# marcinmiklitz/pywindow

Hardware: AMD Instinct MI355X
Metric: trajectory frames/sec full_analysis (pore+windows), CC3 1k-frame (higher is better)
Workload: dtype f64

## Files before the change

pywindow_amd/csrc/pw_unit.hpp:

```cpp
#pragma once
#include "../../include/pywindow_amd.h"
#include "pw_lbfgsb.hpp"
#include "pw_math.hpp"
#include "pw_team.hpp"
#include <string.h>

#if defined(PW_PROFILE) && defined(__HIPCC__)
__shared__ unsigned long long pw_prof_lds[32];
#define PW_PROF_BASE(ws) ((unsigned long long*)pw_prof_lds)
#endif
#if defined(PW_PROFILE) && defined(__HIP_DEVICE_COMPILE__)
#define PW_T0(var) long long var = wall_clock64()
#if defined(PW_ZPROF) && defined(PW_LB_FINE)
#define PW_T1(ws, slot, var) do { (void)var; } while (0)
#elif defined(PW_BARRIER_PROF)
#define PW_T1(ws, slot, var) do { (void)var; if (T::lane() == 0) { unsigned long long w_ = 0; \
        for (int k_ = 0; k_ < T::NWAVES; ++k_) w_ += atomicExch(&pw_bar_acc[k_], 0ull); \
        atomicAdd(&pw_prof_lds[slot], w_); } } while (0)
#else
#define PW_T1(ws, slot, var) do { if (T::lane() == 0) atomicAdd(&pw_prof_lds[slot], (unsigned long long)(wall_clock64() - var)); } while (0)
#endif
#else
#define PW_T0(var) do {} while (0)
#define PW_T1(ws, slot, var) do {} while (0)
#endif

namespace pw {

constexpr double GOLDEN_ANGLE = 2.399963229728653;
constexpr double FOUR_PI = 12.566370614359172;
constexpr double FOUR_THIRDS_PI = 4.1887902047863905;
constexpr double TWO_PI = 6.283185307179586;
constexpr double ONE_PI = 3.141592653589793;

constexpr int PW_KCLS = 8;
#ifndef PW_LEFTOVER_ROUND_DIV
#define PW_LEFTOVER_ROUND_DIV 16
#endif
constexpr double PW_PATH_POINTS_MAX = 1048576.0;
struct ClassInfo {
    int k;
    int off[PW_KCLS + 1];
    double vdw[PW_KCLS];
};
struct Frame {
    ldouble *x, *y, *z, *xx;
    const ldouble* vdw;
    const lint* perm;
    const PW_LDS ClassInfo* cls;
};

struct TeamWorkspace {
    double* knn;
    double* pts;
    double* vals;
    int* surv_k;
    int* labels;
    unsigned char* flag;
    unsigned long long* adj;
    double* xw;
    int* xw_ok;
    int p_cap;
    const unsigned* nb_off;
    const unsigned short* nb_idx;
    const double* nb_unit;
    const double* nb_bound;
    pw_extra_window* xwin;
    unsigned* xwin_count;
    unsigned xwin_cap;
    double leaf[256];
    double acc8[8 * 160];
    int leaf_tab[324];
    unsigned long long prof[32];
    const unsigned* rsq;
    pw_unit_debug* dbg_base;
    long unit;
};
PW_HD inline size_t team_slab_bytes(int p_cap) { return (size_t)p_cap * 192; }
PW_HD inline size_t team_adj_words(int p_cap) { return (size_t)p_cap * (size_t)(p_cap / 64); }
PW_HD inline int round_p_cap(long p) {
    if (p < PW_P_MAX) p = PW_P_MAX;
    return (int)((p + 127) & ~127l);
}
PW_HD inline int params_p_cap(double adjust_windows, double adjust_average) {
    double a = adjust_windows > adjust_average ? adjust_windows : adjust_average;
    if (!(a > 0.0)) a = 1.0;
    double want = 2100.0 * a;
    if (want > 4.0e6) want = 4.0e6;
    return round_p_cap((long)want + 1);
}
PW_HD inline void bind_team_slab(TeamWorkspace* ws, unsigned char* slab, int p_cap) {
    const size_t p = (size_t)p_cap;
    double* d = (double*)slab;
    ws->knn = d; d += 10 * p;
    ws->pts = d; d += 3 * p;
    ws->vals = d; d += p;
    ws->xw = d; d += 7 * p;
    int* i = (int*)d;
    ws->surv_k = i; i += p;
    ws->labels = i; i += p;
    ws->xw_ok = i; i += p;
    ws->flag = (unsigned char*)i;
    ws->p_cap = p_cap;
}

struct UnitVars {
    double com[3];
// ... 66 lines not shown
            bits[0] = (PW_LDS unsigned long long*)p; bits[1] = bits[0] + bw; bits[2] = bits[1] + bw;
            p += 3 * bw * 8;
        }
        ldouble* d = (ldouble*)p;
        vdw = d; d += n;
        mass = d; d += n;
        perm = (lint*)d; d += n / 2;
        inv = (lint*)d; d += n / 2;
        A.x = d; d += n; A.y = d; d += n; A.z = d; d += n; A.xx = d; d += n; A.vdw = vdw; A.perm = perm; A.cls = &v->cls;
        if (nframes > 1) { S.x = d; d += n; S.y = d; d += n; S.z = d; d += n; S.xx = d; d += n; }
        else { S.x = A.x; S.y = A.y; S.z = A.z; S.xx = A.xx; }
        S.vdw = vdw; S.perm = perm; S.cls = &v->cls;
        for (int w = 0; w < 8; ++w) { R[w].x = R[w].y = R[w].z = R[w].xx = nullptr; lb[w] = nullptr; }
        scratch = (PW_LDS unsigned char*)d;
        for (int w = 0; w < nrot; ++w) {
            R[w].x = d; d += n; R[w].y = d; d += n; R[w].z = d; d += n; R[w].xx = d; d += n;
            R[w].vdw = vdw; R[w].perm = perm; R[w].cls = &v->cls;
        }
        rot_words = (size_t)nrot * 4 * n;
        nslots = nrot < nlb ? nrot : nlb;
        p = (PW_LDS unsigned char*)d;
        for (int w = 0; w < nlb; ++w) {
            lb[w] = (PW_LDS void*)p;
            p += (sizeof(LbMem<3>) + 15) & ~(size_t)15;
        }
        scratch_bytes = (size_t)(p - scratch);
    }
};

struct ScratchArena {
    unsigned char* cur;
    size_t left;
    PW_HD void init(const UnitShared& sh) { cur = (unsigned char*)sh.scratch; left = sh.scratch_bytes; }
    PW_HD void* take(size_t bytes) {
        bytes = (bytes + 15) & ~(size_t)15;
        if (bytes > left) return nullptr;
        void* r = cur;
        cur += bytes;
        left -= bytes;
        return r;
    }
};

PW_HD inline void team_atomic_max(PW_LDS int* p, int v) {
#if defined(__HIP_DEVICE_COMPILE__)
    atomicMax((int*)p, v);
#else
    if (v > *p) *p = v;
#endif
}
PW_HD inline void team_atomic_min(int* p, int v) {
#if defined(__HIP_DEVICE_COMPILE__)
    atomicMin(p, v);
#else
    if (v < *p) *p = v;
#endif
}
PW_HD inline void team_atomic_add(int* p, int v) {
#if defined(__HIP_DEVICE_COMPILE__)
    atomicAdd(p, v);
#else
    *p += v;
#endif
}
PW_HD inline unsigned team_atomic_inc(unsigned* p) {
    if (!p) return 0xffffffffu;
#if defined(__HIP_DEVICE_COMPILE__)
    return atomicAdd(p, 1u);
#else
    return __atomic_fetch_add(p, 1u, __ATOMIC_RELAXED);
#endif
}
PW_HD inline void team_atomic_or(PW_LDS unsigned long long* p, unsigned long long v) {
#if defined(__HIP_DEVICE_COMPILE__)
    atomicOr((unsigned long long*)p, v);
#else
    *p |= v;
#endif
}

PW_HD inline double sq3(double a, double b, double c) { return (a * a + c * c) + b * b; }
PW_HD inline double norm3(double a, double b, double c) {
    return pw_sqrt(pw_fma(c, c, pw_fma(b, b, a * a)));
}
PW_HD inline double gap_atom(const Frame& F, int i, double px, double py, double pz, double pp) {
    double g = pw_fma(F.z[i], pz, pw_fma(F.x[i], px, F.y[i] * py));
    double d2 = pw_m2add(g, F.xx[i]) + pp;
    double d = pw_sqrt(d2 > 0.0 ? d2 : 0.0);
    return d - F.vdw[i];
}
PW_HD inline double point_gap(const Frame& F, int n, double px, double py, double pz, int* arg) {
    double pp = sq3(px, py, pz);
    double best = PW_INF;
    int bi = 0x7fffffff;
    for (int i = 0; i < n; ++i) {
        double v = gap_atom(F, i, px, py, pz, pp);
        int oi = F.perm[i];
        if (v < best || (v == best && oi < bi)) { best = v; bi = oi; }
    }
    if (arg) *arg = bi;
    return best;
}
PW_HD inline double point_gap_value(const Frame& F, int n, double px, double py, double pz) {
    const auto& C = *F.cls;
    if (C.k == 0) return point_gap(F, n, px, py, pz, nullptr);
    double pp = sq3(px, py, pz);
    double best = PW_INF;
    for (int g = 0; g < C.k; ++g) {
        double m2 = PW_INF;
        int i = C.off[g];
        const int hi = C.off[g + 1];
        for (; i + 8 <= hi; i += 8) {
            double ax[8], ay[8], az[8], aq[8];
#pragma unroll
            for (int j = 0; j < 8; ++j) { ax[j] = F.x[i + j]; ay[j] = F.y[i + j]; az[j] = F.z[i + j]; aq[j] = F.xx[i + j]; }
#pragma unroll
            for (int j = 0; j < 8; ++j) {
                double gg = pw_fma(az[j], pz, pw_fma(ax[j], px, ay[j] * py));
                m2 = __builtin_fmin(m2, pw_m2add(gg, aq[j]));
            }
        }
        for (; i < hi; ++i) {
            double gg = pw_fma(F.z[i], pz, pw_fma(F.x[i], px, F.y[i] * py));
            m2 = __builtin_fmin(m2, pw_m2add(gg, F.xx[i]));
        }
        m2 = m2 + pp;
        double d = pw_sqrt(m2 > 0.0 ? m2 : 0.0);
        best = __builtin_fmin(best, d - C.vdw[g]);
    }
    return best;
}
template <int NP>
PW_HD inline void points_gap_values(const Frame& F, int n, const double* px, const double* py, const double* pz,
                                    double* out, const lint* cand = nullptr, const lint* coff = nullptr) {
    const auto& C = *F.cls;
    if (C.k == 0) {
        for (int p = 0; p < NP; ++p) out[p] = point_gap(F, n, px[p], py[p], pz[p], nullptr);
        return;
    }
    double qx[NP], qy[NP], qz[NP], pp[NP], best[NP];
#pragma unroll
    for (int p = 0; p < NP; ++p) {
        qx[p] = px[p]; qy[p] = py[p]; qz[p] = pz[p];
        pp[p] = sq3(qx[p], qy[p], qz[p]);
        best[p] = PW_INF;
    }
    for (int g = 0; g < C.k; ++g) {
        double m2[NP];
#pragma unroll
        for (int p = 0; p < NP; ++p) m2[p] = PW_INF;
        if (cand) {
            const int chi = coff[g + 1];
#pragma unroll 4
            for (int c = coff[g]; c < chi; ++c) {
                const int i = cand[c];
                const double x = F.x[i], y = F.y[i], z = F.z[i], xx = F.xx[i];
#pragma unroll
                for (int p = 0; p < NP; ++p) {
                    double gg = pw_fma(z, qz[p], pw_fma(x, qx[p], y * qy[p]));
                    m2[p] = __builtin_fmin(m2[p], pw_m2add(gg, xx));
                }
            }
        } else {
        const int hi = C.off[g + 1];
#pragma unroll 2
        for (int i = C.off[g]; i < hi; ++i) {
// ... 842 lines not shown
    int j = 0;
    while (j + 1 < ConeLatticeTable::N && pw_abs(CONE_LATTICE_TABLE.s[j]) > w) ++j;
    if (j + 1 >= ConeLatticeTable::N) return L;
    double c = (cone_atan2(ry, rx) - delta) / TWO_PI;
    c -= __builtin_floor(c);
    L.c = c < 1.0 ? c : 0.0;
    L.w = w;
    L.j = (short)j;
    return L;
}
struct ConeLatticeWalk {
    double t, w, a, b;
    int k, A, B;
    PW_HD void enter(const ConeLattice& L, int k0, int kend) {
        const int j = L.j, pos = j & 1 ? j + 1 : j, neg = j & 1 ? j : j + 1;
        A = CONE_LATTICE_TABLE.q[pos]; a = CONE_LATTICE_TABLE.s[pos];
        B = CONE_LATTICE_TABLE.q[neg]; b = -CONE_LATTICE_TABLE.s[neg];
        w = L.w;
        k = k0;
        t = (double)k0 * CONE_LATTICE_G - L.c;
        t -= __builtin_floor(t);
        while (k <= kend && !(t < w)) {
            ++k;
            t += CONE_LATTICE_G;
            if (t >= 1.0) t -= 1.0;
        }
    }
    PW_HD void next() {
        if (t + a < w) { k += A; t += a; }
        else if (t - b >= 0.0) { k += B; t -= b; }
        else { k += A + B; t = (t + a) - b; }
    }
};
PW_HD inline ConeLattice* take_cone_lattice(ScratchArena& a, int n) {
#ifdef PW_NO_CONE_LATTICE
    (void)a; (void)n;
    return nullptr;
#else
    return (ConeLattice*)a.take((size_t)(n + 1) * sizeof(ConeLattice));
#endif
}
PW_HD inline __attribute__((always_inline)) int cone_of_atom(double rx, double ry, double rz, double vr, double cn, const Sphere& sp,
                                                            bool narrow, ConeBand* out, ConeLattice* lat_out) {
    const int P = sp.P;
    ConeBand b;
    ConeLattice L;
    L.c = 0.0; L.w = 1.0; L.j = -1; L.first = 0; L.plen = 1;
    int cnt = 0;
    const double rr = sq3(rx, ry, rz);
    const double a2 = rr - pw_fma(rr, 1e-12, (vr * vr) * (1.0 + 1e-12));
    b.klo = 0; b.khi = -P;
    b.thr = -PW_INF;
    if (a2 > 0.0) {
        const double amin = pw_sqrt(a2) * (1.0 - 1e-9);
        b.thr = amin * sp.R * (1.0 - 1e-9);
        if (amin > cn + 1e-6) {
            const double len = pw_sqrt(rr);
            const double zd = rz / len, c = amin / len;
            const double s_ = pw_sqrt(pw_max(1.0 - c * c, 0.0)) * (1.0 + 1e-9) + 1e-9;
            const double rho = pw_sqrt(pw_max(1.0 - zd * zd, 0.0));
            const double zhi = zd >= c ? 1.0 : pw_min(1.0, zd * c + rho * s_ + 1e-9);
            const double zlo = zd <= -c ? -1.0 : pw_max(-1.0, zd * c - rho * s_ - 1e-9);
            const double kh = (zlo - sp.start) / sp.step, kl = (zhi - sp.start) / sp.step;
            b.klo = (int)pw_max(kl - 2.0, 0.0);
            b.khi = (int)pw_min(kh + 3.0, (double)(P - 1));
            if (narrow) {
                L = cone_lattice_window(rx, ry, rz, rr, b.thr, sp.R);
                if (L.j >= 0) {
                    cnt = cone_pieces(b.khi - b.klo + 1, L.w, &L.plen);
                    b.klo = ~b.klo;
                }
            }
        }
    }
    *out = b;
    *lat_out = L;
    return cnt;
}
template <class T, bool FAR, class GETP>
PW_HD inline __attribute__((always_inline)) bool team_ray_tests(const Frame& F, int n, const double* cen, const Sphere& sp,
                                                               GETP getp, ConeBand* bands, unsigned* pairs, int cap,
                                                               PW_LDS int* counts, unsigned char* flag,
                                                               unsigned char hit_value, double* far,
                                                               ConeLattice* lat = nullptr) {
    const int P = sp.P;
    const int seg = cap / T::NWAVES;
    if (P >= 65536 || n >= 65536 || seg < 64) return false;
    const double c0 = cen[0], c1 = cen[1], c2 = cen[2];
    const double cn = norm3(c0, c1, c2);
    int running = 0;
    for (int base = 0; base < n; base += T::SIZE) {
        const int i = base + T::tid();
        ConeBand b;
        ConeLattice L;
        int cnt = 0;
        if (i < n) {
            cnt = cone_of_atom(F.x[i] - c0, F.y[i] - c1, F.z[i] - c2, F.vdw[i], cn, sp, lat != nullptr, &b, &L);
            bands[i] = b;
        }
        if (lat != nullptr) {
            const int inc = T::incl_scan_i(cnt);
            if (T::lane() == T::WSIZE - 1) counts[T::wave()] = inc;
            T::sync();
            int at = running + inc - cnt;
#pragma unroll
            for (int w = 0; w < T::NWAVES; ++w) { const int cw = counts[w]; if (w < T::wave()) at += cw; running += cw; }
            if (i < n) { L.first = at; lat[i] = L; }
            T::sync();
        }
    }
    if (lat != nullptr && T::tid() == 0) lat[n].first = running;
    T::sync();
    int mine = 0;
    unsigned* my = pairs + (size_t)T::wave() * seg;
    auto enumerate = [&](auto bands_, auto lat_, auto my_) __attribute__((always_inline)) {
        for (int g0 = T::wave() * T::WSIZE; g0 < running; g0 += T::SIZE) {
            const int g = g0 + T::lane();
            ConeLatticeWalk wk;
            wk.k = 1;
            int kend = 0, i = 0;
            double rx = 0.0, ry = 0.0, rz = 0.0, thr = 0.0;
            if (g < running) {
                int lo = 0, hi = n - 1;
                while (lo < hi) {
                    const int mid = (lo + hi) >> 1;
                    if (lat_[mid + 1].first > g) hi = mid; else lo = mid + 1;
                }
                i = lo;
                const ConeBand b = bands_[i];
                const ConeLattice L = lat_[i];
                const int k0 = ~b.klo + (g - L.first) * (int)L.plen;
                kend = k0 + (int)L.plen - 1 < b.khi ? k0 + (int)L.plen - 1 : b.khi;
                rx = F.x[i] - c0; ry = F.y[i] - c1; rz = F.z[i] - c2;
                thr = b.thr;
                wk.enter(L, k0, kend);
            }
            while (T::wave_any(wk.k <= kend)) {
                const bool act = wk.k <= kend;
                const int k = wk.k;
                bool f = false;
                if (act) {
                    double px, py, pz;
                    getp(k, &px, &py, &pz);
                    const double dot = pw_fma(pz, rz, pw_fma(px, rx, py * ry));
                    f = dot >= thr;
                    wk.next();
                }
                const unsigned long long bal = T::ballot(f);
                const int pos = mine + __builtin_popcountll(bal & ((1ull << T::lane()) - 1ull));
                if (f && pos < seg) my_[pos] = ((unsigned)k << 16) | (unsigned)i;
                mine += __builtin_popcountll(bal);
            }
        }
    };
    if (lat != nullptr) {
        if (PW_IS_LDS(bands) && PW_IS_LDS(lat) && PW_IS_LDS(my)) enumerate(PW_AS_LDS(bands), PW_AS_LDS(lat), PW_AS_LDS(my));
        else enumerate(bands, lat, my);
    }
    for (int i = T::wave(); i < n; i += T::NWAVES) {
        const ConeBand b = bands[i];
        if (b.klo < 0) continue;
        const bool two_sided = b.khi < 0;
        const int khi = two_sided ? -b.khi - 1 : b.khi;
        const double rx = F.x[i] - c0, ry = F.y[i] - c1, rz = F.z[i] - c2;
        int off = getp.first(b.klo + T::lane());
        for (int kb = b.klo; kb <= khi; kb += T::WSIZE, off += GETP::STEP64) {
            const int k = kb + T::lane();
            bool f = false;
            if (k <= khi) {
                double px, py, pz;
                if (T::WSIZE == 64) getp.at(off, &px, &py, &pz);
                else getp(k, &px, &py, &pz);
                const double dot = pw_fma(pz, rz, pw_fma(px, rx, py * ry));
                f = two_sided ? pw_abs(dot) >= b.thr : dot >= b.thr;
            }
            const unsigned long long bal = T::ballot(f);
            const int pos = mine + __builtin_popcountll(bal & ((1ull << T::lane()) - 1ull));
            if (f && pos < seg) my[pos] = ((unsigned)k << 16) | (unsigned)i;
            mine += __builtin_popcountll(bal);
        }
    }
    if (T::lane() == 0) counts[T::wave()] = mine;
    T::sync();
    int cum[T::NWAVES + 1];
    cum[0] = 0;
    bool fits = true;
#pragma unroll
    for (int w = 0; w < T::NWAVES; ++w) { const int cw = counts[w]; fits = fits && cw <= seg; cum[w + 1] = cum[w] + cw; }
    T::sync();
    if (!fits) return false;
    for (int g = T::tid(); g < cum[T::NWAVES]; g += T::SIZE) {
        int w = 0, first = 0;
#pragma unroll
        for (int q = 1; q < T::NWAVES; ++q)
            if (g >= cum[q]) { w = q; first = cum[q]; }
        const unsigned pr = pairs[(size_t)w * seg + (g - first)];
        const int k = (int)(pr >> 16), i = (int)(pr & 0xffffu);
        double dx, dy, dz;
        getp(k, &dx, &dy, &dz);
        const double nrm = norm3(dx, dy, dz);
        const double ux = dx / nrm, uy = dy / nrm, uz = dz / nrm;
        const double rx = F.x[i] - c0, ry = F.y[i] - c1, rz = F.z[i] - c2;
        const double along = pw_fma(rz, uz, pw_fma(rx, ux, ry * uy));
        const double sq = sq3(rx, ry, rz);
        const double perp = pw_sqrt(sq - along * along);
        const double radicand = F.vdw[i] * F.vdw[i] - perp * perp;
        if (radicand > 0.0) {
            const double half = pw_sqrt(radicand);
            const double tin = along - half, tout = along + half;
            const double ix = c0 + tin * ux, iy = c1 + tin * uy, iz = c2 + tin * uz;
            const double ox = c0 + tout * ux, oy = c1 + tout * uy, oz = c2 + tout * uz;
            const double nin = norm3(ix, iy, iz), nout = norm3(ox, oy, oz);
            if (nin < nout) {
                flag[k] = hit_value;
                if (FAR) team_store_max_pos(&far[k], nout);
            }
        }
    }
    T::sync();
    return true;
}

PW_HD inline double np_floordiv(double a, double b) {
    double mod = __builtin_fmod(a, b);
    double div = (a - mod) / b;
    if (mod != 0.0) {
        if ((b < 0.0) != (mod < 0.0)) div -= 1.0;
    }
    double fl;
    if (div != 0.0) {
        fl = __builtin_floor(div);
        if (div - fl > 0.5) fl += 1.0;
    } else {
        fl = 0.0;
    }
    return fl;
}

PW_NOINLINE PW_HD inline bool path_scan_thread(const Frame& F, int n, double vx, double vy, double vz,
                                   double inc, double m0, double* out_2gap, int* out_pos, double* out_chunk,
                                   int* n_eval, const lint* cand = nullptr, const lint* coff = nullptr) {
    double nrm = norm3(vx, vy, vz);
    int chunks = (int)np_floordiv(nrm, inc);
    double cx = vx / (double)chunks, cy = vy / (double)chunks, cz = vz / (double)chunks;
    double best = PW_INF;
    int pos = 0;
    bool ok = true;
    int k0 = 0;
    if (chunks >= 1) {
        if (!(m0 > 0.0)) ok = false;
        best = m0;
        k0 = 1;
    }
    auto tile = [&](auto np_) __attribute__((always_inline)) {
        constexpr int NP = decltype(np_)::value;
        double qx[NP], qy[NP], qz[NP], m[NP];
#pragma unroll
        for (int p = 0; p < NP; ++p) {
            int k = k0 + p <= chunks ? k0 + p : chunks;
            qx[p] = cx * (double)k; qy[p] = cy * (double)k; qz[p] = cz * (double)k;
        }
        points_gap_values<NP>(F, n, qx, qy, qz, m, cand, coff);
#pragma unroll
        for (int p = 0; p < NP; ++p) {
            if (k0 + p <= chunks && ok) {
                if (!(m[p] > 0.0)) ok = false;
                else if (m[p] < best) { best = m[p]; pos = k0 + p; }
            }
        }
        k0 += NP;
    };
    while (k0 <= chunks && ok) {
        if (chunks - k0 + 1 <= 5) tile(std::integral_constant<int, 5>());
        else tile(std::integral_constant<int, 6>());
    }
    if (n_eval) *n_eval += chunks + 1;
    if (!ok) return false;
    *out_2gap = best * 2.0;
    *out_pos = pos;
    out_chunk[0] = cx; out_chunk[1] = cy; out_chunk[2] = cz;
    return true;
}

struct PathSteps {
    double cx, cy, cz, cd, rinv;
    int chunks;
    bool bracket;
};
PW_HD inline PathSteps path_steps(const Frame& F, double vx, double vy, double vz, double inc, double xx_max) {
    PathSteps s;
    const double nrm = norm3(vx, vy, vz);
    const double fd = np_floordiv(nrm, inc);
    s.bracket = F.cls->k > 0 && fd >= 1.0 && fd <= PW_PATH_POINTS_MAX && nrm < PW_INF;
    s.chunks = s.bracket ? (int)fd : 0;
    s.cd = (double)s.chunks;
    s.cx = vx / s.cd; s.cy = vy / s.cd; s.cz = vz / s.cd;
    const double cc = sq3(s.cx, s.cy, s.cz);
    s.rinv = 1.0 / cc;
    const double bound = (64.0 * 0x1p-53) * (xx_max + sq3(vx, vy, vz));
    s.bracket = s.bracket && cc > 0.0 && cc < PW_INF && s.rinv < PW_INF && bound < PW_INF && cc * (1.0 - 1e-6) > bound;
    return s;
}
PW_NOINLINE PW_HD inline bool path_bracket_thread(const Frame& F, int n, double cx, double cy, double cz, int chunks,
// ... 782 lines not shown
                x1s[c] = xh;
                dxs[c] = xh - xc;
                plain = plain && (dxs[c] != 0.0) && !(xh < lo[c]) && !(xh > up[c]) &&
                        (1e-8 <= pw_max(xc - lo[c], up[c] - xc));
            }
            if (!plain) {
                for (int c = 0; c < 3; ++c) {
                    double xc = c == 0 ? px : (c == 1 ? py : pz);
                    double h = fd_step(xc, lo[c], up[c]);
                    double x1 = xc + h;
                    dxs[c] = x1 - xc;
                    x1s[c] = x1;
                }
            }
            qx[1] = x1s[0]; qy[2] = x1s[1]; qz[3] = x1s[2];
            double gv[4];
            LB_F1(27, f_pre);
#if defined(PW_PROFILE) && defined(PW_LB_FINE) && defined(__HIP_DEVICE_COMPILE__)
            long long t_g4 = clock64();
#endif
#if defined(__HIP_DEVICE_COMPILE__)
            if (T::WSIZE == 64) near_gap.eval(A, n, cand, qx, qy, qz, gv);
            else
#endif
            wave_gap4<T>(A, n, qx, qy, qz, gv);
#if defined(PW_PROFILE) && defined(PW_LB_FINE) && defined(__HIP_DEVICE_COMPILE__)
            if (prof && T::lane() == 0) atomicAdd(&prof[24], (unsigned long long)(clock64() - t_g4));
#endif
            LB_F0(f_post);
            double f0 = -(gv[0] * 2.0);
            for (int c = 0; c < 3; ++c) {
                double f1 = -(gv[c + 1] * 2.0);
                lg[c] = (f1 - f0) / dxs[c];
            }
            lf = f0;
            lx = px; ly = py; lz = pz;
            have_last = true;
            nfev += 4;
            LB_F1(28, f_post);
        }
        fo = lf;
        go[0] = lg[0]; go[1] = lg[1]; go[2] = lg[2];
    }
};

template <class T>
PW_HD inline __attribute__((always_inline)) void stage_opt_impl(UnitShared& sh, TeamWorkspace* ws, int n, pw_unit_out* out,
                                                                const pw_params& prm) {
    (void)ws;
    auto& v = *sh.v;
    if (T::wave() == 0) {
        const Frame A = sh.A;
        Lbfgsb<3> opt;
        Lbfgsb<3>* S = &opt;
        LbMem<3>* Smem = (LbMem<3>*)sh.lb[0];
        PW_ASSUME_LDS(Smem);
        double r = v.pore_g;
        double lo[3], up[3], x0[3];
        int nbd[3] = {2, 2, 2};
        for (int c = 0; c < 3; ++c) x0[c] = (prm.opt_flags & PW_OPT_CUSTOM_START) ? prm.opt_x0[c] : v.com[c];
        if ((prm.opt_flags & PW_OPT_CUSTOM_START) && !(prm.opt_flags & PW_OPT_CUSTOM_BOUNDS))
            r = wave_gap<T>(A, n, x0[0], x0[1], x0[2], nullptr);
        bool bad;
        if (prm.opt_flags & PW_OPT_CUSTOM_BOUNDS) {
            bad = false;
            for (int c = 0; c < 3; ++c) {
                lo[c] = prm.opt_lo[c];
                up[c] = prm.opt_hi[c];
                bool has_lo = lo[c] > -PW_INF, has_up = up[c] < PW_INF;
                nbd[c] = has_lo ? (has_up ? 2 : 1) : (has_up ? 3 : 0);
                if (lo[c] > up[c]) bad = true;
                x0[c] = x0[c] < lo[c] ? lo[c] : (x0[c] > up[c] ? up[c] : x0[c]);
            }
        } else {
            for (int c = 0; c < 3; ++c) {
                lo[c] = x0[c] - r;
                up[c] = x0[c] + r;
            }
            bad = !(r > 0.0);
        }
        int nit = 0, nfev = 0;
        if (!bad) {
            S->template setup<T>(Smem, x0, lo, up, nbd, 1e7, 1e-5, 20);
#if defined(PW_PROFILE) && !defined(PW_ZPROF)
            S->prof = PW_PROF_BASE(ws);
#endif
#if defined(PW_PROFILE) && defined(PW_LB_FINE) && !defined(PW_ZPROF)
            Smem->prof_fine = PW_PROF_BASE(ws);
#endif
            PoreObjective<T> fg(A, n, lo, up, (PW_LDS int*)Smem->cand);
#if defined(PW_PROFILE) && !defined(PW_ZPROF)
            fg.prof = PW_PROF_BASE(ws);
#endif
            PW_T0(t_s);
            S->template minimize<T>(fg, 15000, 15000, &nit);
            T::wave_sync();
            PW_T1(ws, 0, t_s);
            nfev = fg.nfev;
        }
        double cx = v.com[0], cy = v.com[1], cz = v.com[2];
        if (!bad) { cx = S->x[0]; cy = S->x[1]; cz = S->x[2]; }
        int arg;
        double g = wave_gap<T>(A, n, cx, cy, cz, &arg);
        if (T::lane() == 0) {
            v.opt_c[0] = cx; v.opt_c[1] = cy; v.opt_c[2] = cz;
            v.opt_g = g;
            v.opt_atom = arg;
            v.n_eval += nfev + 1;
            if (bad) v.status |= PW_ST_NEGATIVE_PORE;
            out->pore_opt_d = g * 2.0;
            out->pore_opt_atom = arg;
            out->pore_opt_c[0] = cx; out->pore_opt_c[1] = cy; out->pore_opt_c[2] = cz;
            double rr = out->pore_opt_d / 2.0;
            out->pore_vol_opt = FOUR_THIRDS_PI * pw_cube_np(rr);
            out->opt_nit = nit;
            out->opt_nfev = nfev;
            out->opt_task = bad ? -1 : S->task;
            out->opt_msg = bad ? 0 : S->msg;
        }
    }
    T::sync();
}

template <class T>
PW_NOINLINE PW_HD inline void stage_opt(UnitShared& sh, TeamWorkspace* ws, int n, pw_unit_out* out,
                                        const pw_params& prm) {
    stage_opt_impl<T>(sh, ws, n, out, prm);
}

template <class T>
PW_NOINLINE PW_HD inline void stage_average(UnitShared& sh, TeamWorkspace* ws, int n, pw_unit_out* out,
                                             const pw_params& prm) {
    auto& v = *sh.v;
    PW_T0(t_a0);
    make_shifted<T>(sh, n, v.com[0], v.com[1], v.com[2]);
    double keep_d = v.maxd;
    int keep_i = v.maxd_i, keep_j = v.maxd_j;
    T::sync();
    {
        double* ib = 2 * n + 2 <= ws->p_cap ? ws->vals : nullptr;
        team_max_dim<T, true>(sh, sh.S, n, ib);
    }
    double radius = v.maxd;
    T::sync();
    if (T::tid() == 0) { v.maxd = keep_d; v.maxd_i = keep_i; v.maxd_j = keep_j; }
    int P = sampling_count(radius, prm.adjust_average);
    if (P > ws->p_cap) {
        if (T::tid() == 0) { v.status |= PW_ST_POINTS_OVERFLOW; out->avg_d = __builtin_nan(""); out->n_points_avg = P; }
        T::sync();
        return;
    }
    Sphere sp;
    sp.init(radius, P);
    ScratchArena arena;
    arena.init(sh);
    double* vals = (double*)arena.take((size_t)P * 8);
    if (!vals) vals = ws->vals;
    double* packed = vals;
    unsigned char* flag = (unsigned char*)arena.take((size_t)P);
    if (!flag) flag = ws->flag;
    int* s_tab = (int*)arena.take(324 * 4);
    size_t acc_words = 8 * (size_t)(((P < 8192 ? P : 8192) + 63) / 64);
    if (acc_words < 128) acc_words = 128;
    double* s_acc = (double*)arena.take(acc_words * 8);
    double* s_leaf = (double*)arena.take(256 * 8);
    if (!s_tab || !s_acc || !s_leaf) { s_tab = ws->leaf_tab; s_acc = ws->acc8; s_leaf = ws->leaf; }
    double cen[3] = {v.centroid[0], v.centroid[1], v.centroid[2]};
    if (T::wave() == 0) PW_T1(ws, 27, t_a0);
    PW_T0(t_a1);
    bool done = false;
    {
        ScratchArena a2 = arena;
        double* apts = (double*)a2.take((size_t)P * 24);
        if (apts) {
            team_sphere_points<T>(ws, sp, [&](int k, double x, double y, double z) {
                apts[k] = x; apts[P + k] = y; apts[2 * P + k] = z;
                vals[k] = -1.0;
                flag[k] = 0;
            });
            ConeBand* bands = (ConeBand*)a2.take((size_t)n * sizeof(ConeBand));
            ConeLattice* lat = bands ? take_cone_lattice(a2, n) : nullptr;
            int cap = (int)(a2.left / 4);
            unsigned* pairs = (unsigned*)a2.take((size_t)cap * 4);
            if (cap < 4 * P) { pairs = (unsigned*)ws->knn; cap = 16 * ws->p_cap; }
            if (!bands && (size_t)n * sizeof(ConeBand) <= (size_t)ws->p_cap * 16) bands = (ConeBand*)(ws->knn + 8 * (size_t)ws->p_cap);
            PlanarRays<decltype(PW_AS_LDS(apts))> getp{PW_AS_LDS(apts), P};
            if (bands)
                done = team_ray_tests<T, true>(sh.S, n, cen, sp, getp, bands, pairs, cap, (PW_LDS int*)&v.red_i[0], flag, 1, vals, lat);
        }
    }
    if (done) {
    } else if (T::SIZE > 1) {
        constexpr int NR = 4;
        for (int k0 = T::tid(); k0 < P; k0 += NR * T::SIZE) {
            double dx[NR], dy[NR], dz[NR], far[NR];
            bool hit[NR];
#pragma unroll
            for (int r = 0; r < NR; ++r) {
                int k = k0 + r * T::SIZE < P ? k0 + r * T::SIZE : k0;
                sp.point(k, &dx[r], &dy[r], &dz[r]);
            }
            ray_scan_multi<NR>(sh.S, n, cen, dx, dy, dz, hit, far);
#pragma unroll
            for (int r = 0; r < NR; ++r) {
                int k = k0 + r * T::SIZE;
                if (k < P) { vals[k] = far[r]; flag[k] = hit[r] ? 1 : 0; }
            }
        }
    } else {
        for (int k = T::tid(); k < P; k += T::SIZE) {
            double px, py, pz, far;
            sp.point(k, &px, &py, &pz);
            bool hit = ray_scan(sh.S, n, cen, px, py, pz, &far);
            vals[k] = far;
            flag[k] = hit ? 1 : 0;
        }
    }
    T::sync();
    if (T::wave() == 0) PW_T1(ws, 28, t_a1);
    PW_T0(t_a2);
    if (T::wave() == 0) {
        int m = 0;
        for (int base = 0; base < P; base += T::WSIZE) {
            int k = base + T::lane();
            bool f = k < P && flag[k] != 0;
            unsigned long long bal = T::ballot(f);
            int pos = m + __builtin_popcountll(bal & ((1ull << T::lane()) - 1ull));
            if (f) packed[pos] = vals[k];
            m += __builtin_popcountll(bal);
        }
        if (T::lane() == 0) v.n_surv = m;
    }
    T::sync();
    int m = v.n_surv;
    double sum = np_sum_team<T>(packed, m, s_tab, s_acc, s_leaf, &v.red_v[15]);
    if (T::wave() == 0) PW_T1(ws, 29, t_a2);
    if (T::tid() == 0) {
        out->avg_d = (sum / (double)m) * 2.0;
        out->n_points_avg = P;
    }
    T::sync();
}

template <class T>
PW_NOINLINE PW_HD inline void wave_fmin_xy(const Frame& F, int n, double z, double x0, double y0, double* xo,
                               double* yo, int* n_eval) {
    const int maxfun = 400, maxiter = 400;
    const double xatol = 1e-4, fatol = 1e-4;
    double x0s, y0s, f0s, x1s, y1s, f1s, x2s, y2s, f2s;
    int fcalls = 0;
#if defined(__HIP_DEVICE_COMPILE__)
    NearGap1<T> near_gap;
    near_gap.init();
    const Frame Fl = F;
    auto fun = [&](double x, double y) {
        fcalls += 1;
        if (T::WSIZE == 64) return -(near_gap.eval(Fl, n, nullptr, x, y, z) * 2.0);
        return -(wave_gap_value<T>(Fl, n, x, y, z) * 2.0);
    };
#else
    auto fun = [&](double x, double y) {
        fcalls += 1;
        return -(wave_gap_value<T>(F, n, x, y, z) * 2.0);
    };
#endif
    x0s = x0; y0s = y0;
    x1s = (x0 != 0.0) ? (1.0 + 0.05) * x0 : 0.00025; y1s = y0;
    x2s = x0; y2s = (y0 != 0.0) ? (1.0 + 0.05) * y0 : 0.00025;
    f0s = fun(x0s, y0s);
    f1s = fun(x1s, y1s);
    f2s = fun(x2s, y2s);
    auto swap01 = [&]() { double t; t = f0s; f0s = f1s; f1s = t; t = x0s; x0s = x1s; x1s = t; t = y0s; y0s = y1s; y1s = t; };
    auto swap12 = [&]() { double t; t = f1s; f1s = f2s; f2s = t; t = x1s; x1s = x2s; x2s = t; t = y1s; y1s = y2s; y2s = t; };
    auto sort3 = [&]() {
        if (f0s > f1s) swap01();
        if (f1s > f2s) { swap12(); if (f0s > f1s) swap01(); }
    };
    sort3();
    int iterations = 1;
    while (fcalls < maxfun && iterations < maxiter) {
        double dx1 = pw_abs(x1s - x0s), dx2 = pw_abs(x2s - x0s);
        double dy1 = pw_abs(y1s - y0s), dy2 = pw_abs(y2s - y0s);
        double mx = pw_max(pw_max(dx1, dy1), pw_max(dx2, dy2));
        double mf = pw_max(pw_abs(f0s - f1s), pw_abs(f0s - f2s));
        if (mx <= xatol && mf <= fatol) break;
        double bx = (x0s + x1s) / 2.0, by = (y0s + y1s) / 2.0;
        double xr = 2.0 * bx - x2s, yr = 2.0 * by - y2s;
        bool over = false;
        auto guarded = [&](double x, double y, double* f) {
            if (fcalls >= maxfun) { over = true; return false; }
            *f = fun(x, y);
            return true;
        };
        double fxr;
        if (guarded(xr, yr, &fxr)) {
            bool doshrink = false;
            if (fxr < f0s) {
                double xe = 3.0 * bx - 2.0 * x2s, ye = 3.0 * by - 2.0 * y2s;
                double fxe;
                if (guarded(xe, ye, &fxe)) {
                    if (fxe < fxr) { x2s = xe; y2s = ye; f2s = fxe; }
                    else { x2s = xr; y2s = yr; f2s = fxr; }
                }
            } else if (fxr < f1s) {
                x2s = xr; y2s = yr; f2s = fxr;
            } else if (fxr < f2s) {
                double xc = 1.5 * bx - 0.5 * x2s, yc = 1.5 * by - 0.5 * y2s;
                double fxc;
                if (guarded(xc, yc, &fxc)) {
                    if (fxc <= fxr) { x2s = xc; y2s = yc; f2s = fxc; }
                    else doshrink = true;
                }
            } else {
                double xcc = 0.5 * bx + 0.5 * x2s, ycc = 0.5 * by + 0.5 * y2s;
                double fxcc;
                if (guarded(xcc, ycc, &fxcc)) {
// ... 854 lines not shown
                    }
                    auto fill = [&](auto tile_, auto pts_) __attribute__((always_inline)) {
                        if (nb_idx) {
                            const int E0 = s0 + lo, E1 = s0 + hi;
                            const int k1 = (E1 - 1) / 10;
                            for (int k = E0 / 10 + T::tid(); k <= k1; k += T::SIZE) {
                                double d10[10];
                                if (!point_tabled(pts_, k, d10)) {
                                    knn_window_group(pts_, Q4, P, k / NK, W, radius, zstep, ws->knn);
#pragma unroll
                                    for (int q = 0; q < 10; ++q) d10[q] = ws->knn[(size_t)k * 10 + q];
                                }
                                const int e0 = k * 10 - s0;
#pragma unroll
                                for (int q = 0; q < 10; ++q)
                                    if (e0 + q >= lo && e0 + q < hi) tile_[e0 + q - lo] = d10[q];
                            }
                            return;
                        }
                        if (grp >= ngroups) return;
                        for (int p = 0; p < NK; ++p) {
                            const int k = grp * NK + p;
                            const int e0 = e_first + p * 10 - s0;
                            if (k >= P || e0 + 10 <= lo || e0 >= hi) continue;
                            double d10[10];
                            point_dists(pts_, grp, k, searched, d10);
#pragma unroll
                            for (int q = 0; q < 10; ++q)
                                if (e0 + q >= lo && e0 + q < hi) tile_[e0 + q - lo] = d10[q];
                        }
                    };
                    if (PW_IS_LDS(tile) && PW_IS_LDS(pts)) fill(PW_AS_LDS(tile), PW_AS_LDS(pts)); else fill(tile, pts);
                    T::sync();
                    np_leaf_phase<T>(tile, len, lo, hi, s_tab, s_acc, s_leaf, true);
                    lo = hi;
                }
                double part = np_walk_phase<T>(len, s_tab, s_acc, s_leaf);
                if (T::tid() == 0) total = first ? part : total + part;
                first = false;
                T::sync();
            }
            if (T::tid() == 0) v.red_v[15] = total;
            T::sync();
            sum = v.red_v[15];
            T::sync();
        } else {
            sum = np_sum_team<T>(ws->knn, P * 10, s_tab, s_acc, s_leaf, &v.red_v[15]);
        }
        double m = sum / (double)(P * 10);
        if (T::tid() == 0) { v.eps = m + pw_pow_np(m, 0.5); out->eps = v.eps; }
        T::sync();
        if (T::wave() == 0) PW_T1(ws, 25, t_sum);
    }
    if (T::wave() == 0) PW_T1(ws, 8, t_eps);
    PW_T0(t_smp);
    arena = arena_pts;
    double* vals = (double*)arena.take((size_t)P * 8);
    if (!vals) vals = ws->vals;
    int* surv_k = (int*)arena.take((size_t)P * 4);
    if (!surv_k) surv_k = ws->surv_k;
    int* labels = (int*)arena.take((size_t)P * 4);
    if (!labels) labels = ws->labels;
    unsigned char* flag = (unsigned char*)arena.take((size_t)P);
    if (!flag) flag = ws->flag;
    ScratchArena arena_mark = arena;
    double* tmpv = (double*)arena.take((size_t)P * 8);
    if (!tmpv) tmpv = ws->knn;
    {
        double cen[3] = {v.centroid[0], v.centroid[1], v.centroid[2]};
        bool done = false;
        {
            for (int k = T::tid(); k < P; k += T::SIZE) flag[k] = 1;
            ScratchArena a2 = arena_mark;
            ConeBand* bands = (ConeBand*)a2.take((size_t)n * sizeof(ConeBand));
            ConeLattice* lat = bands ? take_cone_lattice(a2, n) : nullptr;
            int cap = (int)(a2.left / 4);
            unsigned* pairs = (unsigned*)a2.take((size_t)cap * 4);
            if (cap < 4 * P) { pairs = (unsigned*)ws->knn; cap = 16 * ws->p_cap; }
            if (!bands && (size_t)n * sizeof(ConeBand) <= (size_t)ws->p_cap * 16) bands = (ConeBand*)(ws->knn + 8 * (size_t)ws->p_cap);
            auto run = [&](auto pts_) __attribute__((always_inline)) {
                SpiralRays<decltype(pts_)> getp{pts_, Q4};
                return team_ray_tests<T, false>(sh.S, n, cen, sp, getp, bands, pairs, cap, (PW_LDS int*)&v.red_i[0], flag, 0, nullptr, lat);
            };
            if (bands) done = PW_IS_LDS(pts) ? run(PW_AS_LDS(pts)) : run(pts);
        }
        if (done) {
        } else if (T::SIZE > 1) {
            constexpr int NR = 4;
            for (int k0 = T::tid(); k0 < P; k0 += NR * T::SIZE) {
                double dx[NR], dy[NR], dz[NR], far[NR];
                bool hit[NR];
#pragma unroll
                for (int r = 0; r < NR; ++r) {
                    int k = k0 + r * T::SIZE < P ? k0 + r * T::SIZE : k0;
                    dx[r] = pts[PT(k, 0)]; dy[r] = pts[PT(k, 1)]; dz[r] = pts[PT(k, 2)];
                }
                ray_scan_multi<NR, false>(sh.S, n, cen, dx, dy, dz, hit, far);
#pragma unroll
                for (int r = 0; r < NR; ++r) {
                    int k = k0 + r * T::SIZE;
                    if (k < P) flag[k] = hit[r] ? 0 : 1;
                }
            }
        } else {
            for (int k = T::tid(); k < P; k += T::SIZE) {
                double far;
                bool hit = ray_scan(sh.S, n, cen, pts[PT(k, 0)], pts[PT(k, 1)], pts[PT(k, 2)], &far);
                flag[k] = hit ? 0 : 1;
            }
        }
        T::sync();
        if (T::wave() == 0) {
            int m = 0;
            for (int base = 0; base < P; base += T::WSIZE) {
                int k = base + T::lane();
                bool f = k < P && flag[k] != 0;
                unsigned long long bal = T::ballot(f);
                int pos = m + __builtin_popcountll(bal & ((1ull << T::lane()) - 1ull));
                if (f) labels[pos] = k;
                m += __builtin_popcountll(bal);
            }
            if (T::lane() == 0) v.n_surv = m;
        }
        T::sync();
        int ncand = v.n_surv;
        int evals = 0;
        if (T::wave() == 0) PW_T1(ws, 30, t_smp);
        PW_T0(t_path);
        const double m_origin = wave_gap_value<T>(sh.S, n, 0.0, 0.0, 0.0);
        int whole = T::SIZE > 1 ? (ncand / T::SIZE) * T::SIZE : ncand;
        if ((ncand - whole) * PW_LEFTOVER_ROUND_DIV >= T::SIZE) whole = ncand;
        lint* cand_w = nullptr;
        lint* coff_w = nullptr;
        {
            ScratchArena a3 = arena;
            const size_t per_wave = (size_t)n + PW_KCLS + 2;
            int* c_all = (int*)a3.take((size_t)T::NWAVES * per_wave * 4);
#ifndef PW_NO_SCAN_LISTS
            if (c_all && PW_IS_LDS(c_all)) {
                cand_w = (lint*)PW_AS_LDS(c_all) + (size_t)T::wave() * per_wave;
                coff_w = cand_w + n;
            }
#endif
        }
#ifndef PW_NO_PATH_BRACKETS
        double xx_max = 0.0;
        if (ncand > 0) {
            for (int i = T::lane(); i < n; i += T::WSIZE) xx_max = __builtin_fmax(xx_max, sh.S.xx[i]);
            xx_max = -T::wave_min(-xx_max);
        }
#endif
        for (int j0 = 0; j0 < whole; j0 += T::SIZE) {
            const int j = j0 + T::tid();
            const bool have = j < whole;
            const int k = have ? labels[j] : 0;
            const double vx = pts[PT(k, 0)], vy = pts[PT(k, 1)], vz = pts[PT(k, 2)];
            const bool listed = cand_w != nullptr &&
                                wave_path_candidates<T>(sh.S, n, have, vx, vy, vz, prm.increment, m_origin, cand_w, coff_w);
#ifndef PW_NO_PATH_BRACKETS
            const PathSteps steps = path_steps(sh.S, vx, vy, vz, prm.increment, xx_max);
            if (!T::wave_any(have && !steps.bracket)) {
                if (have) {
                    double g2 = 0.0;
                    bool ok = path_bracket_thread(sh.S, n, steps.cx, steps.cy, steps.cz, steps.chunks, steps.rinv, m_origin,
                                                  &g2, &evals, listed ? cand_w : nullptr, listed ? coff_w : nullptr);
                    flag[j] = ok ? 1 : 0;
                    tmpv[j] = g2;
                }
                continue;
            }
#endif
            if (have) {
                double g2, chunk[3];
                int pos;
                bool ok = path_scan_thread(sh.S, n, vx, vy, vz, prm.increment, m_origin, &g2, &pos, chunk, &evals,
                                           listed ? cand_w : nullptr, listed ? coff_w : nullptr);
                flag[j] = ok ? 1 : 0;
                tmpv[j] = g2;
            }
        }
        const int left = ncand - whole;
        if (left > 0) {
            for (int j = whole + T::wave(); j < ncand; j += T::NWAVES) {
                const int k = labels[j];
                const double vx = pts[PT(k, 0)], vy = pts[PT(k, 1)], vz = pts[PT(k, 2)];
                const int chunks = (int)np_floordiv(norm3(vx, vy, vz), prm.increment);
                double g2 = 0.0;
                bool ok = true;
                bool bracketed = false;
#ifndef PW_NO_PATH_BRACKETS
                {
                    const PathSteps steps = path_steps(sh.S, vx, vy, vz, prm.increment, xx_max);
                    if (steps.bracket) {
                        const PathMin pm = wave_path_bracket<T>(sh.S, n, steps.cx, steps.cy, steps.cz, steps.chunks, steps.rinv, 1);
                        ok = m_origin > 0.0 && pm.gap > 0.0;
                        if (ok) g2 = (pm.gap < m_origin ? pm.gap : m_origin) * 2.0;
                        bracketed = true;
                    }
                }
#endif
                if (bracketed) {
                } else if (chunks >= 1) {
                    const double cx = vx / (double)chunks, cy = vy / (double)chunks, cz = vz / (double)chunks;
                    double best = m_origin;
                    if (!(m_origin > 0.0)) ok = false;
                    for (int q = 1; q <= chunks && ok; ++q) {
                        const double m = wave_gap_value<T>(sh.S, n, cx * (double)q, cy * (double)q, cz * (double)q);
// ... 233 lines not shown
```

Baseline: 1.065 million.

## Pre-normalize ray directions, compare squared norms, and parallelize flag compaction across waves

Sphere sample points are normalized once when they are generated, so the per-pair ray test skips the norm and three divisions, and cone thresholds are rescaled to match. The inside/outside comparison now uses squared norms, with an exact sqrt fallback only when the two values are nearly equal, so most pairs avoid two square roots. Survivor compaction changes from a single-wave ballot loop to a two-pass scan that uses every wave. The risks are small floating-point differences in threshold decisions (guarded by a 1e-9 margin) and an extra barrier in the compaction. Optional profiling macros are added as well.

New measurement: 1.070 million, median of 6. No clear change (+0.5%).

```diff
diff --git a/pywindow_amd/csrc/pw_unit.hpp b/pywindow_amd/csrc/pw_unit.hpp
--- a/pywindow_amd/csrc/pw_unit.hpp
+++ b/pywindow_amd/csrc/pw_unit.hpp
@@ -23,6 +23,11 @@
 #else
 #define PW_T0(var) do {} while (0)
 #define PW_T1(ws, slot, var) do {} while (0)
+#endif
+#if defined(PW_PROFILE) && defined(PW_RAY_PROF) && !defined(PW_LB_FINE) && !defined(PW_ZPROF)
+#define PW_TR(slot, var) do { if (T::wave() == 0) PW_T1(nullptr, slot, var); } while (0)
+#else
+#define PW_TR(slot, var) do {} while (0)
 #endif
 
 namespace pw {
@@ -255,6 +260,22 @@
 PW_HD inline double sq3(double a, double b, double c) { return (a * a + c * c) + b * b; }
 PW_HD inline double norm3(double a, double b, double c) {
     return pw_sqrt(pw_fma(c, c, pw_fma(b, b, a * a)));
+}
+PW_HD inline double norm3_arg(double a, double b, double c) { return pw_fma(c, c, pw_fma(b, b, a * a)); }
+#if defined(PW_RAY_UNIT_STATS) && !defined(__HIPCC__)
+inline unsigned long long ray_unit_stats[2] = {0, 0};
+#define PW_RAY_UNIT_COUNT(slot) (++ray_unit_stats[slot])
+#else
+#define PW_RAY_UNIT_COUNT(slot) ((void)0)
+#endif
+PW_HD inline bool roots_less(double a, double b) {
+    PW_RAY_UNIT_COUNT(0);
+#ifndef PW_NO_RAY_UNITS
+    if (a >= b) return false;
+    if (b > a * (1.0 + 0x1p-49)) return true;
+#endif
+    PW_RAY_UNIT_COUNT(1);
+    return pw_sqrt(a) < pw_sqrt(b);
 }
 PW_HD inline double gap_atom(const Frame& F, int i, double px, double py, double pz, double pp) {
     double g = pw_fma(F.z[i], pz, pw_fma(F.x[i], px, F.y[i] * py));
@@ -1263,12 +1284,14 @@
                                                                GETP getp, ConeBand* bands, unsigned* pairs, int cap,
                                                                PW_LDS int* counts, unsigned char* flag,
                                                                unsigned char hit_value, double* far,
-                                                               ConeLattice* lat = nullptr) {
+                                                               ConeLattice* lat = nullptr, bool unit = false) {
     const int P = sp.P;
     const int seg = cap / T::NWAVES;
     if (P >= 65536 || n >= 65536 || seg < 64) return false;
     const double c0 = cen[0], c1 = cen[1], c2 = cen[2];
     const double cn = norm3(c0, c1, c2);
+    const double thr_scale = unit ? (1.0 / sp.R) * (1.0 - 1e-9) : 1.0;
+    PW_T0(t_cones);
     int running = 0;
     for (int base = 0; base < n; base += T::SIZE) {
         const int i = base + T::tid();
@@ -1277,6 +1300,7 @@
         int cnt = 0;
         if (i < n) {
             cnt = cone_of_atom(F.x[i] - c0, F.y[i] - c1, F.z[i] - c2, F.vdw[i], cn, sp, lat != nullptr, &b, &L);
+            b.thr *= thr_scale;
             bands[i] = b;
         }
         if (lat != nullptr) {
@@ -1292,6 +1316,8 @@
     }
     if (lat != nullptr && T::tid() == 0) lat[n].first = running;
     T::sync();
+    PW_TR(16, t_cones);
+    PW_T0(t_enum);
     int mine = 0;
     unsigned* my = pairs + (size_t)T::wave() * seg;
     auto enumerate = [&](auto bands_, auto lat_, auto my_) __attribute__((always_inline)) {
@@ -1338,6 +1364,8 @@
         if (PW_IS_LDS(bands) && PW_IS_LDS(lat) && PW_IS_LDS(my)) enumerate(PW_AS_LDS(bands), PW_AS_LDS(lat), PW_AS_LDS(my));
         else enumerate(bands, lat, my);
     }
+    PW_TR(17, t_enum);
+    PW_T0(t_walk);
     for (int i = T::wave(); i < n; i += T::NWAVES) {
         const ConeBand b = bands[i];
         if (b.klo < 0) continue;
@@ -1369,6 +1397,8 @@
 #pragma unroll
     for (int w = 0; w < T::NWAVES; ++w) { const int cw = counts[w]; fits = fits && cw <= seg; cum[w + 1] = cum[w] + cw; }
     T::sync();
+    PW_TR(18, t_walk);
+    PW_T0(t_pairs);
     if (!fits) return false;
     for (int g = T::tid(); g < cum[T::NWAVES]; g += T::SIZE) {
         int w = 0, first = 0;
@@ -1379,8 +1409,11 @@
         const int k = (int)(pr >> 16), i = (int)(pr & 0xffffu);
         double dx, dy, dz;
         getp(k, &dx, &dy, &dz);
-        const double nrm = norm3(dx, dy, dz);
-        const double ux = dx / nrm, uy = dy / nrm, uz = dz / nrm;
+        double ux = dx, uy = dy, uz = dz;
+        if (!unit) {
+            const double nrm = norm3(dx, dy, dz);
+            ux = dx / nrm; uy = dy / nrm; uz = dz / nrm;
+        }
         const double rx = F.x[i] - c0, ry = F.y[i] - c1, rz = F.z[i] - c2;
         const double along = pw_fma(rz, uz, pw_fma(rx, ux, ry * uy));
         const double sq = sq3(rx, ry, rz);
@@ -1391,15 +1424,44 @@
             const double tin = along - half, tout = along + half;
             const double ix = c0 + tin * ux, iy = c1 + tin * uy, iz = c2 + tin * uz;
             const double ox = c0 + tout * ux, oy = c1 + tout * uy, oz = c2 + tout * uz;
-            const double nin = norm3(ix, iy, iz), nout = norm3(ox, oy, oz);
-            if (nin < nout) {
+            const double ain = norm3_arg(ix, iy, iz), aout = norm3_arg(ox, oy, oz);
+            if (roots_less(ain, aout)) {
                 flag[k] = hit_value;
-                if (FAR) team_store_max_pos(&far[k], nout);
-            }
-        }
-    }
-    T::sync();
+                if (FAR) team_store_max_pos(&far[k], pw_sqrt(aout));
+            }
+        }
+    }
+    T::sync();
+    PW_TR(19, t_pairs);
     return true;
+}
+
+template <class T, class PUT>
+PW_HD inline __attribute__((always_inline)) int team_compact_flags(const unsigned char* flag, int P, PW_LDS int* counts,
+                                                                  int* n_out, PUT put) {
+    const int per = ((P + T::SIZE - 1) / T::SIZE) * T::WSIZE;
+    const int lo = T::wave() * per;
+    const int hi = lo + per < P ? lo + per : P;
+    const unsigned long long below = (1ull << T::lane()) - 1ull;
+    int cnt = 0;
+    for (int base = lo; base < hi; base += T::WSIZE) {
+        const int k = base + T::lane();
+        cnt += __builtin_popcountll(T::ballot(k < hi && flag[k] != 0));
+    }
+    if (T::lane() == 0) counts[T::wave()] = cnt;
+    T::sync();
+    int m = 0, total = 0;
+#pragma unroll
+    for (int w = 0; w < T::NWAVES; ++w) { const int cw = counts[w]; if (w < T::wave()) m += cw; total += cw; }
+    for (int base = lo; base < hi; base += T::WSIZE) {
+        const int k = base + T::lane();
+        const bool f = k < hi && flag[k] != 0;
+        const unsigned long long bal = T::ballot(f);
+        if (f) put(m + __builtin_popcountll(bal & below), k);
+        m += __builtin_popcountll(bal);
+    }
+    if (T::tid() == 0) *n_out = total;
+    return total;
 }
 
 PW_HD inline double np_floordiv(double a, double b) {
@@ -2348,7 +2410,7 @@
         int nit = 0, nfev = 0;
         if (!bad) {
             S->template setup<T>(Smem, x0, lo, up, nbd, 1e7, 1e-5, 20);
-#if defined(PW_PROFILE) && !defined(PW_ZPROF)
+#if defined(PW_PROFILE) && !defined(PW_ZPROF) && !defined(PW_RAY_PROF)
             S->prof = PW_PROF_BASE(ws);
 #endif
 #if defined(PW_PROFILE) && defined(PW_LB_FINE) && !defined(PW_ZPROF)
@@ -2435,11 +2497,21 @@
     if (T::wave() == 0) PW_T1(ws, 27, t_a0);
     PW_T0(t_a1);
     bool done = false;
+    double* apts = nullptr;
     {
         ScratchArena a2 = arena;
-        double* apts = (double*)a2.take((size_t)P * 24);
+        apts = (double*)a2.take((size_t)P * 24);
         if (apts) {
+#ifndef PW_NO_RAY_UNITS
+            const bool unit = true;
+#else
+            const bool unit = false;
+#endif
             team_sphere_points<T>(ws, sp, [&](int k, double x, double y, double z) {
+                if (unit) {
+                    const double nrm = norm3(x, y, z);
+                    x = x / nrm; y = y / nrm; z = z / nrm;
+                }
                 apts[k] = x; apts[P + k] = y; apts[2 * P + k] = z;
                 vals[k] = -1.0;
                 flag[k] = 0;
@@ -2451,8 +2523,9 @@
             if (cap < 4 * P) { pairs = (unsigned*)ws->knn; cap = 16 * ws->p_cap; }
             if (!bands && (size_t)n * sizeof(ConeBand) <= (size_t)ws->p_cap * 16) bands = (ConeBand*)(ws->knn + 8 * (size_t)ws->p_cap);
             PlanarRays<decltype(PW_AS_LDS(apts))> getp{PW_AS_LDS(apts), P};
+            PW_TR(20, t_a1);
             if (bands)
-                done = team_ray_tests<T, true>(sh.S, n, cen, sp, getp, bands, pairs, cap, (PW_LDS int*)&v.red_i[0], flag, 1, vals, lat);
+                done = team_ray_tests<T, true>(sh.S, n, cen, sp, getp, bands, pairs, cap, (PW_LDS int*)&v.red_i[0], flag, 1, vals, lat, unit);
         }
     }
     if (done) {
@@ -2485,7 +2558,15 @@
     T::sync();
     if (T::wave() == 0) PW_T1(ws, 28, t_a1);
     PW_T0(t_a2);
-    if (T::wave() == 0) {
+#ifndef PW_NO_RAY_UNITS
+    const bool team_compaction = done;
+#else
+    const bool team_compaction = false;
+#endif
+    if (team_compaction) {
+        packed = apts;
+        team_compact_flags<T>(flag, P, (PW_LDS int*)&v.red_i[0], &v.n_surv, [&](int pos, int k) { packed[pos] = vals[k]; });
+    } else if (T::wave() == 0) {
         int m = 0;
         for (int base = 0; base < P; base += T::WSIZE) {
             int k = base + T::lane();
@@ -2498,6 +2579,7 @@
         if (T::lane() == 0) v.n_surv = m;
     }
     T::sync();
+    PW_TR(21, t_a2);
     int m = v.n_surv;
     double sum = np_sum_team<T>(packed, m, s_tab, s_acc, s_leaf, &v.red_v[15]);
     if (T::wave() == 0) PW_T1(ws, 29, t_a2);
@@ -3518,6 +3600,7 @@
                 SpiralRays<decltype(pts_)> getp{pts_, Q4};
                 return team_ray_tests<T, false>(sh.S, n, cen, sp, getp, bands, pairs, cap, (PW_LDS int*)&v.red_i[0], flag, 0, nullptr, lat);
             };
+            PW_TR(22, t_smp);
             if (bands) done = PW_IS_LDS(pts) ? run(PW_AS_LDS(pts)) : run(pts);
         }
         if (done) {
@@ -3546,7 +3629,15 @@
             }
         }
         T::sync();
-        if (T::wave() == 0) {
+        PW_T0(t_cmp);
+#ifndef PW_NO_RAY_UNITS
+        const bool team_compaction = true;
+#else
+        const bool team_compaction = false;
+#endif
+        if (team_compaction) {
+            team_compact_flags<T>(flag, P, (PW_LDS int*)&v.red_i[0], &v.n_surv, [&](int pos, int k) { labels[pos] = k; });
+        } else if (T::wave() == 0) {
             int m = 0;
             for (int base = 0; base < P; base += T::WSIZE) {
                 int k = base + T::lane();
@@ -3559,6 +3650,7 @@
             if (T::lane() == 0) v.n_surv = m;
         }
         T::sync();
+        PW_TR(22, t_cmp);
         int ncand = v.n_surv;
         int evals = 0;
         if (T::wave() == 0) PW_T1(ws, 30, t_smp);
```
